# mrlooi/PoseCNN

Measured on AMD Instinct MI355X. Metric: frames/sec 640x480x21-class Hough-vote+RoI+ADD-loss, 1/2/4/8 MI355X, higher is better.
Workload: dtype f32 (FC GEMMs: exact 3-way split-bf16 x6 MFMA, products within 2^-24, fp32 accumulate: fp32-faithful)

## Files before the change

posecnn_amd/average_distance_loss/average_distance_loss_op.py:

```python
import warnings

import torch

from .. import _lib


def workspace_bytes(R, num_classes, num_points):
    return _lib.load().pcnn_add_loss_workspace_size(R, num_classes, num_points)


def search_stats(workspace, R, num_classes, num_points):
    off = _lib.load().pcnn_add_loss_stats_offset(R, num_classes, num_points)
    f, s, t = workspace[off:off + 12].cpu().view(torch.int32).tolist()
    return {"filter_items": f, "scan_items": s, "triples": t, "exact_evals": 16 * t}


def _workspace(what, ws, R, C, P):
    _lib.require(ws, torch.uint8, name=f"{what}: workspace")
    need = workspace_bytes(R, C, P)
    if ws.numel() < need:
        raise ValueError(f"{what}: workspace must hold {need} bytes, got {ws.numel()}")


def _models(what, points, symmetry, C, normalise):
    if normalise:
        points, symmetry = points.contiguous().float(), symmetry.contiguous().float()
    if points.dim() != 3 or points.shape[0] != C or points.shape[2] != 3:
        raise ValueError(f"{what}: points must be ({C}, P, 3), got {tuple(points.shape)}")
    _lib.require(points, torch.float32, name=f"{what}: points")
    _lib.require(symmetry, torch.float32, name=f"{what}: symmetry")
    if symmetry.numel() != C:
        raise ValueError(f"{what}: symmetry must have {C} elements, got {symmetry.numel()}")
    return points, symmetry


def average_distance_loss_prep(bottom_weight, bottom_symmetry, num_points, workspace, num_rois=None, points=None):
    if points is not None:
        warnings.warn("average_distance_loss_prep: `points` is ignored (the pruned ADD-S search is removed)",
                      DeprecationWarning, stacklevel=2)
    _lib.require_gpu(bottom_weight, bottom_symmetry, workspace)
    if bottom_weight.dim() != 2 or bottom_weight.shape[1] % 4:
        raise ValueError("average_distance_loss_prep: weight must be (R, 4C)")
    w = bottom_weight.contiguous().float()
    R, PC = w.shape
    sym = bottom_symmetry.contiguous().float()
    if sym.numel() != PC // 4:
        raise ValueError(f"average_distance_loss_prep: symmetry must have {PC // 4} elements, got {sym.numel()}")
    _workspace("average_distance_loss_prep", workspace, R, PC // 4, int(num_points))
    _lib.require_counter(num_rois, "average_distance_loss_prep: num_rois")
    rc = _lib.load().pcnn_add_loss_prep(_lib.ptr(w), _lib.ptr(sym), R,
                                        _lib.ptr(num_rois), PC // 4, int(num_points), _lib.ptr(workspace),
                                        workspace.numel(), _lib.stream_ptr())
    _lib.check(rc, "average_distance_loss_prep")


def average_distance_loss(bottom_prediction, bottom_target, bottom_weight, bottom_point, bottom_symmetry, margin,
                          name=None, num_rois=None, loss_norm_rows=0, loss_norm_rows_dev=None, out=None,
                          workspace=None, prepared=False):
    _lib.require_gpu(bottom_prediction, bottom_target, bottom_weight, bottom_point, bottom_symmetry)
    if margin < 0:
        raise ValueError(f"Need margin >= 0, got {margin}")
    what = "average_distance_loss"
    if bottom_prediction.dim() != 2 or bottom_prediction.shape[1] % 4:
        raise ValueError(f"{what}: prediction must be (R, 4C)")
    pred = bottom_prediction.contiguous().float()
    R, PC = pred.shape
    C = PC // 4
    for name, t in (("target", bottom_target), ("weight", bottom_weight)):
        if tuple(t.shape) != (R, PC):
            raise ValueError(f"{what}: {name} must be {(R, PC)} as the prediction, got {tuple(t.shape)}")
    points, symmetry = _models(what, bottom_point, bottom_symmetry, C, normalise=True)
    P = points.shape[1]
    _lib.require_counter(num_rois, f"{what}: num_rois")
    _lib.require_counter(loss_norm_rows_dev, f"{what}: loss_norm_rows_dev")
    if workspace is not None:
        _workspace(what, workspace, R, C, P)
    lib = _lib.load()
    if prepared and workspace is None:
        raise ValueError("prepared=True needs the workspace average_distance_loss_prep wrote")
    ws = workspace if workspace is not None else _lib.workspace(lib.pcnn_add_loss_workspace_size(R, C, P),
                                                                pred.device, "add_loss")
    if out is None:
        loss = torch.empty((1,), dtype=torch.float32, device=pred.device)
        diff = torch.empty((R, PC), dtype=torch.float32, device=pred.device)
    else:
        loss, diff = out
        _lib.require(loss, torch.float32, shape=(1,), name=f"{what}: out[0] (loss)")
        _lib.require(diff, torch.float32, shape=(R, PC), name=f"{what}: out[1] (bottom_diff)")
    fn = lib.pcnn_add_loss_fwd_prepared if prepared else lib.pcnn_add_loss_fwd
    rc = fn(_lib.ptr(pred), _lib.ptr(bottom_target.contiguous().float()), _lib.ptr(bottom_weight.contiguous().float()),
            _lib.ptr(points), _lib.ptr(symmetry), R,
            _lib.ptr(num_rois), C, P, float(margin), int(loss_norm_rows), _lib.ptr(loss_norm_rows_dev), _lib.ptr(loss),
            _lib.ptr(diff), _lib.ptr(ws), ws.numel(), _lib.stream_ptr())
    _lib.check(rc, "average_distance_loss")
    return loss, diff


def average_distance_loss_head_bwd(pred, target, weight, points, symmetry, margin, tanh_out, d_pred_scale, diff, dy8,
                                   workspace, num_rois=None, loss_norm_rows_dev=None, checked=True):
    _lib.require_gpu(pred, target, weight, points, symmetry, tanh_out, diff, dy8, workspace)
    what = "average_distance_loss_head_bwd"
    if margin < 0:
        raise ValueError(f"Need margin >= 0, got {margin}")
    if pred.dim() != 2 or pred.shape[1] % 4:
        raise ValueError(f"{what}: pred must be (R, 4C)")
    R, PC = pred.shape
    if PC > 256:
        raise ValueError(f"{what}: at most 256 columns (4C), got {PC}")
    _models(what, points, symmetry, PC // 4, normalise=False)
    if checked:
        for name, t in (("pred", pred), ("target", target), ("weight", weight), ("tanh_out", tanh_out),
                        ("diff", diff), ("dy8", dy8)):
            _lib.require(t, torch.float32, shape=(R, PC), name=f"{what}: {name}")
        if d_pred_scale is not None and _lib.require(d_pred_scale, torch.float32,
                                                     name=f"{what}: d_pred_scale").numel() < 1:
            raise ValueError(f"{what}: d_pred_scale needs one element")
        _workspace(what, workspace, R, PC // 4, points.shape[1])
        _lib.require_counter(num_rois, f"{what}: num_rois")
        _lib.require_counter(loss_norm_rows_dev, f"{what}: loss_norm_rows_dev")
    rc = _lib.load().pcnn_add_loss_fwd_head_bwd(
        _lib.ptr(pred), _lib.ptr(target), _lib.ptr(weight), _lib.ptr(points), _lib.ptr(symmetry), R,
        _lib.ptr(num_rois), PC // 4, points.shape[1], float(margin), 0, _lib.ptr(loss_norm_rows_dev), _lib.ptr(diff),
        _lib.ptr(workspace), workspace.numel(), _lib.ptr(tanh_out), _lib.ptr(d_pred_scale), _lib.ptr(dy8),
        _lib.stream_ptr())
    _lib.check(rc, "average_distance_loss_head_bwd")


def average_distance_loss_total(R, num_classes, num_points, workspace, loss, num_rois=None, checked=True):
    _lib.require_gpu(workspace, loss)
    if checked:
        _workspace("average_distance_loss_total", workspace, R, num_classes, num_points)
        _lib.require(loss, torch.float32, shape=(1,), name="average_distance_loss_total: loss")
        _lib.require_counter(num_rois, "average_distance_loss_total: num_rois")
    rc = _lib.load().pcnn_add_loss_total(R, _lib.ptr(num_rois), num_classes, num_points, _lib.ptr(workspace),
                                         workspace.numel(), _lib.ptr(loss), _lib.stream_ptr())
    _lib.check(rc, "average_distance_loss_total")


def average_distance_loss_grad(bottom_diff, grad, margin=0.01, name=None, num_rois=None, out=None):
    _lib.require_gpu(bottom_diff, grad)
    bd = bottom_diff.contiguous().float()
    g = grad.contiguous().float()
    if g.numel() < 1:
        raise ValueError("average_distance_loss_grad: grad needs one element")
    o = out if out is not None else torch.empty_like(bd)
    if out is not None:
        _lib.require(out, torch.float32, shape=tuple(bd.shape), name="average_distance_loss_grad: out")
    _lib.require_counter(num_rois, "average_distance_loss_grad: num_rois")
    rc = _lib.load().pcnn_add_loss_bwd(_lib.ptr(g), _lib.ptr(bd), bd.numel(),
                                       _lib.ptr(num_rois), bd.shape[-1], _lib.ptr(o), _lib.stream_ptr())
    _lib.check(rc, "average_distance_loss_grad")
    return o


class AverageDistanceFunction(torch.autograd.Function):

    @staticmethod
    def forward(ctx, pred, target, weight, points, symmetry, margin):
        loss, diff = average_distance_loss(pred, target, weight, points, symmetry, margin)
        ctx.save_for_backward(diff)
        ctx.margin = margin
        return loss

    @staticmethod
    def backward(ctx, grad):
        (diff,) = ctx.saved_tensors
        return average_distance_loss_grad(diff, grad.reshape(1), ctx.margin), None, None, None, None, None
```

posecnn_amd/csrc/average_distance.hip:

```cpp
#include "pcnn_common.h"
#include "head_common.h"
#include <atomic>
#include <cfloat>
#include <cstdlib>
#include <cstring>
#include <type_traits>

namespace {

#ifndef ADD_LANES
#define ADD_LANES 64
#endif
constexpr int kSymLanes = ADD_LANES;
#ifndef ADD_GRID
#define ADD_GRID 1024
#endif
#ifndef ADD_PPL
#define ADD_PPL 4
#endif
constexpr int kPPL = ADD_PPL;
constexpr int kPts = kSymLanes * kPPL;
constexpr int kMaxPointsLds = 8192;

__device__ __forceinline__ int rows_of(const int32_t* dev, int cap) {
  if (!dev) return cap;
  int r = *dev;
  return r < cap ? r : cap;
}

__device__ __forceinline__ void quat2rot(float s, float u, float v, float w, float* r) {
  r[0] = s * s + u * u - v * v - w * w;
  r[1] = 2 * (u * v - s * w);
  r[2] = 2 * (u * w + s * v);
  r[3] = 2 * (u * v + s * w);
  r[4] = s * s - u * u + v * v - w * w;
  r[5] = 2 * (v * w - s * u);
  r[6] = 2 * (u * w - s * v);
  r[7] = 2 * (v * w + s * u);
  r[8] = s * s - u * u - v * v + w * w;
}

__device__ __forceinline__ float div_rn(float x, float b, float r) {
  const float y0 = x * r;
  const float y1 = fmaf(fmaf(-y0, b, x), r, y0);
  return fmaf(fmaf(-y1, b, x), r, y1);
}
__device__ __forceinline__ double div_rn(double x, double b, double r) {
  const double y0 = x * r;
  const double y1 = fma(fma(-y0, b, x), r, y0);
  return fma(fma(-y1, b, x), r, y1);
}

__global__ void k_div_rn_check(const float* __restrict__ x, float b, int n, int dbl, float* __restrict__ out) {
  const int i = blockIdx.x * blockDim.x + threadIdx.x;
  if (i >= n) return;
  if (dbl) {
    const double bd = (double)b, rd = 1.0 / bd;
    out[i] = (float)div_rn((double)x[i], bd, rd);
  } else {
    out[i] = div_rn(x[i], b, 1.f / b);
  }
}

__device__ __forceinline__ int row_class(const float* __restrict__ weight, int n, int C) {
  const float* w = weight + (size_t)n * 4 * C;
  for (int i0 = 0; i0 < C; i0 += 8) {
    float v[8];
#pragma unroll
    for (int j = 0; j < 8; j++) v[j] = i0 + j < C ? w[4 * (i0 + j)] : 0.f;
#pragma unroll
    for (int j = 0; j < 8; j++)
      if (v[j] > 0) return i0 + j;
  }
  return -1;
}

__device__ __forceinline__ void add_point_terms(float X0, float X1, float X2, float x1, float y1, float z1, float x2,
                                                float y2, float z2, float s, float u, float v, float w, float margin,
                                                float bn, float rbn, double ln, double rln, float* acc) {
  const float dist = (x1 - x2) * (x1 - x2) + (y1 - y2) * (y1 - y2) + (z1 - z2) * (z1 - z2);
  if (dist < margin) return;
  acc[0] += (float)div_rn((double)(dist - margin), ln, rln);
  const float d0[9] = {2 * s, -2 * w, 2 * v, 2 * w, 2 * s, -2 * u, -2 * v, 2 * u, 2 * s};
  const float d1[9] = {2 * u, 2 * v, 2 * w, 2 * v, -2 * u, -2 * s, 2 * w, 2 * s, -2 * u};
  const float d2[9] = {-2 * v, 2 * u, 2 * s, 2 * u, 2 * v, 2 * w, -2 * s, 2 * w, -2 * v};
  const float d3[9] = {-2 * w, -2 * s, 2 * u, 2 * s, -2 * w, 2 * v, 2 * u, 2 * v, 2 * w};
  const float X[3] = {X0, X1, X2};
  const float df[3] = {x1 - x2, y1 - y2, z1 - z2};
  float e0 = 0.f, e1 = 0.f, e2 = 0.f, e3 = 0.f;
#pragma unroll
  for (int a = 0; a < 3; a++)
#pragma unroll
    for (int b = 0; b < 3; b++) {
      e0 += div_rn(df[a] * X[b] * d0[a * 3 + b], bn, rbn);
      e1 += div_rn(df[a] * X[b] * d1[a * 3 + b], bn, rbn);
      e2 += div_rn(df[a] * X[b] * d2[a * 3 + b], bn, rbn);
      e3 += div_rn(df[a] * X[b] * d3[a * 3 + b], bn, rbn);
    }
  acc[1] += e0; acc[2] += e1; acc[3] += e2; acc[4] += e3;
}

template <int kRows>
__device__ __forceinline__ void add_plain_rows(int n0, const float* __restrict__ pred,
                                               const float* __restrict__ target, const float* __restrict__ points,
                                               const float* __restrict__ symmetry, int R, int C, int P, float margin,
                                               int norm_rows, const int32_t* __restrict__ norm_rows_dev, int nchunk,
                                               const int32_t* __restrict__ rcls, float* __restrict__ partial,
                                               float (*red)[5]) {
  const int half = kRows == 2 ? (int)(threadIdx.x / kPts) : 0, tid = (int)(threadIdx.x % kPts);
  const int n = n0 + half;
  const bool live = n < R;
  const int cls = live ? rcls[n] : -1;
  const bool sym = cls >= 0 && symmetry[cls] > 0;
  float* out = partial + (size_t)(live ? n : 0) * nchunk * 5;
  if (live && !sym)
    for (int i = tid; i < nchunk * 5; i += kPts) out[i] = 0.f;
  const bool work = live && !sym && cls >= 0;
  float acc[5] = {0.f, 0.f, 0.f, 0.f, 0.f};
  if (work) {
    const int PC = 4 * C;
    const float* tq = target + (size_t)n * PC + 4 * cls;
    const float* pq = pred + (size_t)n * PC + 4 * cls;
    float Rg[9], Rp[9];
    quat2rot(tq[0], tq[1], tq[2], tq[3], Rg);
    const float s = pq[0], u = pq[1], v = pq[2], w = pq[3];
    quat2rot(s, u, v, w, Rp);
    const int Rn = norm_rows_dev ? *norm_rows_dev : (norm_rows > 0 ? norm_rows : R);
    const float bn = (float)(Rn * P), rbn = 1.f / bn;
    const double ln = 2.0 * (double)Rn * (double)P, rln = 1.0 / ln;
    const float* pts = points + (size_t)cls * P * 3;
    for (int p = tid; p < P; p += kPts) {
      const float X0 = pts[p * 3 + 0], X1 = pts[p * 3 + 1], X2 = pts[p * 3 + 2];
      const float x1 = Rp[0] * X0 + Rp[1] * X1 + Rp[2] * X2;
      const float y1 = Rp[3] * X0 + Rp[4] * X1 + Rp[5] * X2;
      const float z1 = Rp[6] * X0 + Rp[7] * X1 + Rp[8] * X2;
      const float x2 = Rg[0] * X0 + Rg[1] * X1 + Rg[2] * X2;
      const float y2 = Rg[3] * X0 + Rg[4] * X1 + Rg[5] * X2;
      const float z2 = Rg[6] * X0 + Rg[7] * X1 + Rg[8] * X2;
      add_point_terms(X0, X1, X2, x1, y1, z1, x2, y2, z2, s, u, v, w, margin, bn, rbn, ln, rln, acc);
    }
  }
#pragma unroll
  for (int q = 0; q < 5; q++) acc[q] = pcnn::wave_sum(acc[q]);
  if (pcnn::lane_id() == 0)
    for (int q = 0; q < 5; q++) red[threadIdx.x >> 6][q] = acc[q];
  __syncthreads();
  if (work && tid < 5) {
    float t = 0.f;
    for (int i = 0; i < kPts / 64; i++) t += red[half * (kPts / 64) + i][tid];
    out[tid] = t;
  }
}

#ifndef ADD_GROUPS
#define ADD_GROUPS 4
#endif
constexpr int kSymGroups = ADD_GROUPS;
constexpr int kSymThreads = kSymLanes * kSymGroups;
#ifndef ADD_BLK
#define ADD_BLK 8
#endif
constexpr int kBlk = ADD_BLK;

typedef unsigned u32x4 __attribute__((ext_vector_type(4)));
typedef float f32x16 __attribute__((ext_vector_type(16)));
typedef __bf16 bf16x8 __attribute__((ext_vector_type(8)));

constexpr int kFiltWaves = 8;
constexpr int kFiltThreads = 64 * kFiltWaves;
constexpr int kFiltMaxPoints = 2816;
constexpr int kFiltList = 1024;
constexpr int kFiltBlk = ((kFiltMaxPoints + 31) / 32 + kFiltWaves - 1) / kFiltWaves;
constexpr float kFiltWin = 2.8e-4f;
constexpr float kFiltM2Min = 0x1p-40f, kFiltM2Max = 0x1p40f;
constexpr unsigned kFiltPadNorm = 0x7180u;

template <bool F>
struct FiltLds {};
template <>
struct FiltLds<true> {
  float4 sq[kPts];
  float smin[kFiltWaves][kPts];
  unsigned long long skey[kPts];
  unsigned list[kFiltList];
  int cnt, m2;
};

__device__ __forceinline__ unsigned bf16_rn(float x) {
  const unsigned b = __float_as_uint(x);
  return (b + 0x7fffu + ((b >> 16) & 1u)) >> 16;
}
__device__ __forceinline__ float bf16_val(unsigned h) { return __uint_as_float(h << 16); }
__device__ __forceinline__ void bf16_split2(float x, unsigned& h, unsigned& m) {
  h = bf16_rn(x);
  m = bf16_rn(x - bf16_val(h));
}

__device__ __forceinline__ void filt_candidate(const float4& c, float n, u32x4& k0, u32x4& k8) {
  unsigned xh, xm, yh, ym, zh, zm;
  bf16_split2(c.x, xh, xm);
  bf16_split2(c.y, yh, ym);
  bf16_split2(c.z, zh, zm);
  const unsigned nh = bf16_rn(n);
  const float r1 = n - bf16_val(nh);
  const unsigned nm = bf16_rn(r1);
  const unsigned nl = bf16_rn(r1 - bf16_val(nm));
  k0 = (u32x4){xh | xh << 16, xm | xm << 16, yh | yh << 16, ym | ym << 16};
  k8 = (u32x4){zh | zh << 16, zm | zm << 16, nh | nm << 16, nl};
}

__device__ __forceinline__ float filt_min17(float m, const f32x16& v) {
  float a = fminf(fminf(v[0], v[1]), v[2]);
  float b = fminf(fminf(v[3], v[4]), v[5]);
  a = fminf(fminf(a, v[6]), v[7]);
  b = fminf(fminf(b, v[8]), v[9]);
  a = fminf(fminf(a, v[10]), v[11]);
  b = fminf(fminf(b, v[12]), v[13]);
  a = fminf(fminf(a, v[14]), v[15]);
  return fminf(fminf(m, a), b);
}

template <int NF>
__device__ __forceinline__ int filter_search(FiltLds<true>& fl, const float4* gpts, const char* cimg, int P, int nq,
                                             float win, int* s_imin) {
  const int lane = pcnn::lane_id(), r = lane & 31, h = lane >> 5;
  const int wave = __builtin_amdgcn_readfirstlane((int)(threadIdx.x >> 6));
  const int nblk = (P + 31) >> 5, bq = nblk / kFiltWaves, brem = nblk % kFiltWaves;
  const int b0 = wave * bq + min(wave, brem), b1 = b0 + bq + (wave < brem ? 1 : 0);
  bf16x8 qb[NF];
#pragma unroll
  for (int f = 0; f < NF; f++) {
    const float4 q = fl.sq[f * 32 + r];
    unsigned xh, xm, yh, ym, zh, zm;
    bf16_split2(-2.f * q.x, xh, xm);
    bf16_split2(-2.f * q.y, yh, ym);
    bf16_split2(-2.f * q.z, zh, zm);
    const u32x4 w = h == 0 ? (u32x4){xh | xm << 16, xh | xm << 16, yh | ym << 16, yh | ym << 16}
                           : (u32x4){zh | zm << 16, zh | zm << 16, 0x3f803f80u, 0x00003f80u};
    qb[f] = __builtin_bit_cast(bf16x8, w);
  }
  const f32x16 zero = {0.f, 0.f, 0.f, 0.f, 0.f, 0.f, 0.f, 0.f, 0.f, 0.f, 0.f, 0.f, 0.f, 0.f, 0.f, 0.f};
  const char* ap = cimg + r * 32 + h * 16;
  float bmin[kFiltBlk][NF];
  bf16x8 a = *(const bf16x8*)(ap + min(b0, nblk - 1) * 1024);
#pragma unroll
  for (int k = 0; k < kFiltBlk; k++) {
    if (b0 + k < b1) {
      const bf16x8 an = *(const bf16x8*)(ap + min(b0 + k + 1, nblk - 1) * 1024);
      f32x16 v = __builtin_amdgcn_mfma_f32_32x32x16_bf16(a, qb[0], zero, 0, 0, 0);
#pragma unroll
      for (int f = 0; f < NF; f++) {
        f32x16 vn = v;
        if (f + 1 < NF) vn = __builtin_amdgcn_mfma_f32_32x32x16_bf16(a, qb[f + 1], zero, 0, 0, 0);
        __builtin_amdgcn_sched_barrier(0);
        bmin[k][f] = filt_min17(FLT_MAX, v);
        __builtin_amdgcn_sched_barrier(0);
        v = vn;
      }
      a = an;
    } else {
#pragma unroll
      for (int f = 0; f < NF; f++) bmin[k][f] = FLT_MAX;
    }
  }
#pragma unroll
  for (int f = 0; f < NF; f++) {
    float m = bmin[0][f];
#pragma unroll
    for (int k = 1; k < kFiltBlk; k++) m = fminf(m, bmin[k][f]);
    m = fminf(m, __shfl_xor(m, 32, 64));
    if (h == 0) fl.smin[wave][f * 32 + r] = m;
  }
  __syncthreads();
  unsigned mask[NF];
#pragma unroll
  for (int f = 0; f < NF; f++) {
    float t = fl.smin[0][f * 32 + r];
#pragma unroll
    for (int g = 1; g < kFiltWaves; g++) t = fminf(t, fl.smin[g][f * 32 + r]);
    const float thr = t + win;
    unsigned mk = 0u;
#pragma unroll
    for (int k = 0; k < kFiltBlk; k++) mk |= bmin[k][f] <= thr ? 1u << k : 0u;
    mask[f] = mk;
  }
#pragma unroll
  for (int f = 0; f < NF; f++)
    if (f * 32 + r >= nq) mask[f] = 0u;
  int nrec = 0;
  for (;;) {
    int mine = 0;
#pragma unroll
    for (int f = 0; f < NF; f++) mine += __popc(mask[f]);
    int incl = mine;
#pragma unroll
    for (int o = 1; o < 64; o <<= 1) {
      const int t = __shfl_up(incl, o, 64);
      if (lane >= o) incl += t;
    }
    const int total = __shfl(incl, 63, 64);
    int base = 0;
    if (lane == 0 && total > 0) base = atomicAdd(&fl.cnt, total);
    int pos = __shfl(base, 0, 64) + incl - mine;
    int pending = 0;
#pragma unroll
    for (int f = 0; f < NF; f++) {
      unsigned mk = mask[f];
      while (mk && pos < kFiltList) {
        const int bit = __ffs(mk) - 1;
        mk &= mk - 1;
        fl.list[pos++] = (unsigned)(f * 32 + r) << 16 | (unsigned)(b0 + bit) << 1 | (unsigned)h;
      }
      mask[f] = mk;
      pending |= mk != 0u;
    }
    __syncthreads();
    const int n = min(fl.cnt, kFiltList);
    for (int w = threadIdx.x; w < n; w += blockDim.x) {
      const unsigned rec = fl.list[w];
      const int qi = rec >> 16;
      const int i0 = (int)((rec >> 1) & 0x7fffu) * 32 + 4 * (int)(rec & 1u);
      const float4 q = fl.sq[qi];
      unsigned long long best = ~0ull;
#pragma unroll
      for (int reg = 0; reg < 16; reg++) {
        const int idx = i0 + (reg & 3) + 8 * (reg >> 2);
        const float4 c = gpts[min(idx, P - 1)];
        const float d = (q.x - c.x) * (q.x - c.x) + (q.y - c.y) * (q.y - c.y) + (q.z - c.z) * (q.z - c.z);
        const unsigned long long key = (unsigned long long)__float_as_uint(d) << 32 | (unsigned long long)(unsigned)idx;
        if (idx < P && d < FLT_MAX && key < best) best = key;
      }
      if (best != ~0ull) atomicMin(&fl.skey[qi], best);
    }
    nrec += n;
    pending = __syncthreads_or(pending);
    if (!pending) break;
    if (threadIdx.x == 0) fl.cnt = 0;
    __syncthreads();
  }
  if (threadIdx.x < kPts) {
    const unsigned long long key = fl.skey[threadIdx.x];
    s_imin[threadIdx.x] = key == ~0ull ? -1 : (int)(unsigned)(key & 0xffffffffull);
  }
  return nrec;
}

template <bool kFilt>
__global__ void __launch_bounds__(kFilt ? kFiltThreads : kSymThreads) k_add_rows(const float* __restrict__ pred,
                                                           const float* __restrict__ target,
                                                           const float* __restrict__ weight,
                                                           const float* __restrict__ points,
                                                           const float* __restrict__ symmetry, int R_cap,
                                                           const int32_t* __restrict__ num_rois_dev, int C, int P,
                                                           float margin, int norm_rows,
                                                           const int32_t* __restrict__ norm_rows_dev, int nchunk,
                                                           const int32_t* __restrict__ rcls,
                                                           const int32_t* __restrict__ sym_rows,
                                                           const int32_t* __restrict__ nsym,
                                                           int32_t* __restrict__ queue,
                                                           int32_t* __restrict__ stats,
                                                           float* __restrict__ partial) {
  extern __shared__ __attribute__((aligned(16))) float4 gpts[];
  __shared__ FiltLds<kFilt> fl;
  __shared__ float mdist[kSymGroups - 1][kPts];
  __shared__ int midx[kSymGroups - 1][kPts];
  __shared__ float red[(kFilt ? kFiltThreads : kSymThreads) / 64][5];
  __shared__ int s_imin[kPts];
  const int R = rows_of(num_rois_dev, R_cap);
  const int sym_items = *nsym * nchunk;
  constexpr int kPlain = kFilt ? kFiltThreads / kPts : 1;
  const int items = sym_items + (R + kPlain - 1) / kPlain;
  const int grp = threadIdx.x / kSymLanes, lt = threadIdx.x % kSymLanes;
  const int quarter = ((P + kSymGroups - 1) / kSymGroups + kBlk - 1) / kBlk * kBlk;
  const int c0 = grp * quarter, c1 = min(P, c0 + quarter);
  __shared__ int s_item;
  int st_filter = 0, st_scan = 0, st_triples = 0;
  for (;;) {
  __syncthreads();
  if (threadIdx.x == 0) {
    s_item = atomicAdd(queue, 1);
    if constexpr (kFilt) { fl.cnt = 0; fl.m2 = 0; }
  }
  __syncthreads();
  const int item = s_item;
  if (item >= items) break;
  if (item >= sym_items) {
    add_plain_rows<kPlain>((item - sym_items) * kPlain, pred, target, points, symmetry, R, C, P, margin, norm_rows,
                           norm_rows_dev, nchunk, rcls, partial, red);
    continue;
  }
  const int nfull = P / kPts, nsym_rows = *nsym;
  int n, chunk, slot;
  if (item < nsym_rows * nfull) {
    slot = item / nfull;
    chunk = item % nfull;
  } else {
    slot = item - nsym_rows * nfull;
    chunk = nfull;
  }
  n = sym_rows[slot];
  const int PC = 4 * C;
  const int cls = rcls[n];
  float* out = partial + ((size_t)n * nchunk + chunk) * 5;
  const float* tq = target + (size_t)n * PC + 4 * cls;
  const float* pq = pred + (size_t)n * PC + 4 * cls;
  float Rg[9], Rp[9];
  quat2rot(tq[0], tq[1], tq[2], tq[3], Rg);
  const float s = pq[0], u = pq[1], v = pq[2], w = pq[3];
  quat2rot(s, u, v, w, Rp);
  const float* pts = points + (size_t)cls * P * 3;
  const int nq = min(kPts, P - chunk * kPts);
  bool searched = false;
  int nrec = 0;
  float Xt0 = 0.f, Xt1 = 0.f, Xt2 = 0.f;
  if constexpr (kFilt) {
    char* cimg = (char*)gpts + (((size_t)P * sizeof(float4) + 31) & ~(size_t)31);
    const int Ppad = (P + 31) & ~31;
    float mx = 0.f;
    int bad = 0;
    constexpr int kStage = (kFiltMaxPoints + kFiltThreads - 1) / kFiltThreads;
    float Xs[kStage][3];
#pragma unroll
    for (int k = 0; k < kStage; k++) {
      const int i = (int)threadIdx.x + k * kFiltThreads;
      const int ii = i < P ? i : 0;
      Xs[k][0] = pts[ii * 3 + 0]; Xs[k][1] = pts[ii * 3 + 1]; Xs[k][2] = pts[ii * 3 + 2];
    }
#pragma unroll
    for (int k = 0; k < kStage; k++) {
      const int i = (int)threadIdx.x + k * kFiltThreads;
      if (i >= Ppad) continue;
      u32x4 k0 = {0u, 0u, 0u, 0u}, k8 = {0u, 0u, kFiltPadNorm, 0u};
      if (i < P) {
        const float X0 = Xs[k][0], X1 = Xs[k][1], X2 = Xs[k][2];
        const float4 c = make_float4(Rg[0] * X0 + Rg[1] * X1 + Rg[2] * X2, Rg[3] * X0 + Rg[4] * X1 + Rg[5] * X2,
                                     Rg[6] * X0 + Rg[7] * X1 + Rg[8] * X2, 0.f);
        gpts[i] = c;
        const float nn = c.x * c.x + c.y * c.y + c.z * c.z;
        bad |= !(nn <= kFiltM2Max);
        mx = fmaxf(mx, nn);
        filt_candidate(c, nn, k0, k8);
      }
      *(u32x4*)(cimg + (size_t)i * 32) = k0;
      *(u32x4*)(cimg + (size_t)i * 32 + 16) = k8;
    }
    if (threadIdx.x < kPts) {
      const int p = chunk * kPts + (int)threadIdx.x;
      const int pp = p < P ? p : 0;
      const float X0 = pts[pp * 3 + 0], X1 = pts[pp * 3 + 1], X2 = pts[pp * 3 + 2];
      Xt0 = X0; Xt1 = X1; Xt2 = X2;
      const float4 q = make_float4(Rp[0] * X0 + Rp[1] * X1 + Rp[2] * X2, Rp[3] * X0 + Rp[4] * X1 + Rp[5] * X2,
                                   Rp[6] * X0 + Rp[7] * X1 + Rp[8] * X2, 0.f);
      fl.sq[threadIdx.x] = q;
      const float nn = q.x * q.x + q.y * q.y + q.z * q.z;
      bad |= !(nn <= kFiltM2Max);
      mx = fmaxf(mx, nn);
      fl.skey[threadIdx.x] = ~0ull;
    }
    mx = pcnn::wave_max(mx);
    if (pcnn::lane_id() == 0) atomicMax(&fl.m2, __float_as_int(mx));
    bad = __syncthreads_or(bad);
    const float m2 = __int_as_float(fl.m2);
    if (!bad && m2 >= kFiltM2Min) {
      nrec = nq > 64 ? filter_search<8>(fl, gpts, cimg, P, nq, kFiltWin * m2, s_imin)
                     : filter_search<2>(fl, gpts, cimg, P, nq, kFiltWin * m2, s_imin);
      searched = true;
    }
  } else {
  for (int i = threadIdx.x; i < P; i += blockDim.x) {
    const float X0 = pts[i * 3 + 0], X1 = pts[i * 3 + 1], X2 = pts[i * 3 + 2];
    gpts[i] = make_float4(Rg[0] * X0 + Rg[1] * X1 + Rg[2] * X2, Rg[3] * X0 + Rg[4] * X1 + Rg[5] * X2,
                          Rg[6] * X0 + Rg[7] * X1 + Rg[8] * X2, 0.f);
  }
  __syncthreads();
  }
  if (!searched) {
  float qx[kPPL], qy[kPPL], qz[kPPL], Xq[kPPL][3];
  int pq_[kPPL];
#pragma unroll
  for (int k = 0; k < kPPL; k++) {
    const int p = chunk * kPts + k * kSymLanes + lt;
    pq_[k] = p;
    const int pp = p < P ? p : 0;
    Xq[k][0] = pts[pp * 3 + 0]; Xq[k][1] = pts[pp * 3 + 1]; Xq[k][2] = pts[pp * 3 + 2];
    qx[k] = Rp[0] * Xq[k][0] + Rp[1] * Xq[k][1] + Rp[2] * Xq[k][2];
    qy[k] = Rp[3] * Xq[k][0] + Rp[4] * Xq[k][1] + Rp[5] * Xq[k][2];
    qz[k] = Rp[6] * Xq[k][0] + Rp[7] * Xq[k][1] + Rp[8] * Xq[k][2];
  }
  auto dist_to = [&](int k, const float4& c) {
    return (qx[k] - c.x) * (qx[k] - c.x) + (qy[k] - c.y) * (qy[k] - c.y) + (qz[k] - c.z) * (qz[k] - c.z);
  };
  float dmin[kPPL];
  int iblk[kPPL];
#pragma unroll
  for (int k = 0; k < kPPL; k++) { dmin[k] = FLT_MAX; iblk[k] = -1; }
  typedef float f2 __attribute__((ext_vector_type(2)));
  f2 px[kPPL / 2], py[kPPL / 2], pz[kPPL / 2];
#pragma unroll
  for (int h = 0; h < kPPL / 2; h++) {
    px[h] = (f2){qx[2 * h], qx[2 * h + 1]};
    py[h] = (f2){qy[2 * h], qy[2 * h + 1]};
    pz[h] = (f2){qz[2 * h], qz[2 * h + 1]};
  }
  auto scan = [&](auto np_c) {
    constexpr int NP = decltype(np_c)::value;
    int i = c0;
    for (; i + kBlk <= c1; i += kBlk) {
      float4 c[kBlk];
#pragma unroll
      for (int j = 0; j < kBlk; j++) c[j] = gpts[i + j];
#pragma unroll
      for (int h = 0; h < NP; h++) {
        f2 d[kBlk];
#pragma unroll
        for (int j = 0; j < kBlk; j++) {
          const f2 ex = px[h] - c[j].x, ey = py[h] - c[j].y, ez = pz[h] - c[j].z;
          d[j] = ex * ex + ey * ey + ez * ez;
        }
#pragma unroll
        for (int e = 0; e < 2; e++) {
          const int k = 2 * h + e;
          float bm = fminf(d[0][e], d[1][e]);
#pragma unroll
          for (int j = 2; j < kBlk; j += 2) bm = fminf(bm, fminf(d[j][e], d[j + 1][e]));
          if (bm < dmin[k]) { dmin[k] = bm; iblk[k] = i; }
        }
      }
    }
    for (; i < c1; i++) {
      const float4 c = gpts[i];
#pragma unroll
      for (int k = 0; k < 2 * NP; k++) {
        const float d = dist_to(k, c);
        if (d < dmin[k]) { dmin[k] = d; iblk[k] = i; }
      }
    }
  };
  if (nq > 2 * kSymLanes) scan(std::integral_constant<int, kPPL / 2>{});
  else scan(std::integral_constant<int, 1>{});
  if (grp > 0 && grp < kSymGroups) {
#pragma unroll
    for (int k = 0; k < kPPL; k++) {
      mdist[grp - 1][k * kSymLanes + lt] = dmin[k];
      midx[grp - 1][k * kSymLanes + lt] = iblk[k];
    }
  }
  __syncthreads();
  if (grp == 0) {
#pragma unroll
    for (int k = 0; k < kPPL; k++) {
#pragma unroll
      for (int g = 0; g < kSymGroups - 1; g++) {
        const float d = mdist[g][k * kSymLanes + lt];
        if (d < dmin[k]) { dmin[k] = d; iblk[k] = midx[g][k * kSymLanes + lt]; }
      }
      int im = -1;
      if (iblk[k] >= 0) {
        const int e = min(iblk[k] + kBlk, P);
        for (int j = iblk[k]; j < e; j++)
          if (dist_to(k, gpts[j]) == dmin[k]) { im = j; break; }
      }
      s_imin[k * kSymLanes + lt] = im;
    }
  }
  }
  __syncthreads();
  float acc[5] = {0.f, 0.f, 0.f, 0.f, 0.f};
  for (int jj = threadIdx.x; jj < kPts; jj += blockDim.x) {
    const int p = chunk * kPts + jj;
    if (p >= P) continue;
    const int im = s_imin[jj] < 0 ? p : s_imin[jj];
    static_assert(kPts == kSymThreads, "one tail point per thread: jj == threadIdx.x");
    const float X0 = kFilt ? Xt0 : pts[p * 3 + 0], X1 = kFilt ? Xt1 : pts[p * 3 + 1], X2 = kFilt ? Xt2 : pts[p * 3 + 2];
    const float x1 = Rp[0] * X0 + Rp[1] * X1 + Rp[2] * X2;
    const float y1 = Rp[3] * X0 + Rp[4] * X1 + Rp[5] * X2;
    const float z1 = Rp[6] * X0 + Rp[7] * X1 + Rp[8] * X2;
    const float4 cm = gpts[im];
    const int Rn = norm_rows_dev ? *norm_rows_dev : (norm_rows > 0 ? norm_rows : R);
    const float bn = (float)(Rn * P), rbn = 1.f / bn;
    const double ln = 2.0 * (double)Rn * (double)P, rln = 1.0 / ln;
    add_point_terms(X0, X1, X2, x1, y1, z1, cm.x, cm.y, cm.z, s, u, v, w, margin, bn, rbn, ln, rln, acc);
  }
#pragma unroll
  for (int q = 0; q < 5; q++) acc[q] = pcnn::wave_sum(acc[q]);
  if (pcnn::lane_id() == 0 && threadIdx.x < kSymThreads)
    for (int q = 0; q < 5; q++) red[threadIdx.x >> 6][q] = acc[q];
  __syncthreads();
  if (threadIdx.x < 5) {
    float t = 0.f;
    for (int i = 0; i < kSymThreads / 64; i++) t += red[i][threadIdx.x];
    out[threadIdx.x] = t;
  }
  if (searched) {
    st_filter++;
    st_triples += nrec;
  } else {
    st_scan++;
  }
  __syncthreads();
  }
  if (threadIdx.x == 0) {
    if (st_filter) atomicAdd(stats + 0, st_filter);
    if (st_scan) atomicAdd(stats + 1, st_scan);
    if (st_triples) atomicAdd(stats + 2, st_triples);
  }
}

__global__ void __launch_bounds__(1024) k_add_prep(const float* __restrict__ weight, const float* __restrict__ symmetry,
                                                    int R_cap, const int32_t* __restrict__ num_rois_dev, int C,
                                                    int32_t* __restrict__ rcls, int32_t* __restrict__ sym_rows,
                                                    int32_t* __restrict__ nsym, int32_t* __restrict__ queue,
                                                    int32_t* __restrict__ stats) {
  __shared__ int wcount[16];
  __shared__ int base;
  const int R = rows_of(num_rois_dev, R_cap);
  const int lane = pcnn::lane_id(), wave = threadIdx.x >> 6;
  if (threadIdx.x == 0) base = 0;
  __syncthreads();
  for (int n0 = 0; n0 < R; n0 += blockDim.x) {
    const int n = n0 + threadIdx.x;
    int cls = -1;
    if (n < R) {
      cls = row_class(weight, n, C);
      rcls[n] = cls;
    }
    const bool sym = n < R && cls >= 0 && symmetry[cls] > 0;
    const uint64_t m = __ballot(sym);
    if (lane == 0) wcount[wave] = __popcll(m);
    __syncthreads();
    int off = base;
    for (int w = 0; w < wave; w++) off += wcount[w];
    if (sym) sym_rows[off + __popcll(m & pcnn::lanemask_lt())] = n;
    __syncthreads();
    if (threadIdx.x == 0) {
      int t = 0;
      for (int w = 0; w < (int)(blockDim.x >> 6); w++) t += wcount[w];
      base += t;
    }
    __syncthreads();
  }
  if (threadIdx.x == 0) {
    *nsym = base;
    *queue = 0;
    stats[0] = stats[1] = stats[2] = 0;
  }
}

__device__ __forceinline__ void fold_row(int n, int nchunk, const float* __restrict__ partial, int lane, float* s) {
#pragma unroll
  for (int q = 0; q < 5; q++) s[q] = 0.f;
  for (int k = lane; k < nchunk; k += 64)
    for (int q = 0; q < 5; q++) s[q] += partial[((size_t)n * nchunk + k) * 5 + q];
#pragma unroll
  for (int q = 0; q < 5; q++) s[q] = pcnn::wave_sum(s[q]);
}

__device__ __forceinline__ void finish_row(int n, int R, int C, int nchunk, const int32_t* __restrict__ rcls,
                                           const float* __restrict__ partial, float* __restrict__ row_loss,
                                           float* __restrict__ bottom_diff, int lane) {
  if (n >= R) return;
  const int cls = rcls[n];
  float s[5];
  fold_row(n, nchunk, partial, lane, s);
  const int PC = 4 * C;
  for (int col = lane; col < PC; col += 64) {
    float vv = 0.f;
    if (cls >= 0 && col >= 4 * cls && col < 4 * cls + 4) vv = s[1 + col - 4 * cls];
    bottom_diff[(size_t)n * PC + col] = vv;
  }
  if (lane == 0) row_loss[n] = cls >= 0 ? s[0] : 0.f;
}

__global__ void __launch_bounds__(256) k_add_finish_rows(int R_cap, const int32_t* __restrict__ num_rois_dev, int C,
                                                          int nchunk, const int32_t* __restrict__ rcls,
                                                          const float* __restrict__ partial,
                                                          float* __restrict__ row_loss,
                                                          float* __restrict__ bottom_diff) {
  const int R = rows_of(num_rois_dev, R_cap);
  const int n = (blockIdx.x * blockDim.x + threadIdx.x) >> 6;
  finish_row(n, R, C, nchunk, rcls, partial, row_loss, bottom_diff, pcnn::lane_id());
}

__global__ void __launch_bounds__(256) k_add_finish_head(int R_cap, const int32_t* __restrict__ num_rois_dev, int C,
                                                          int nchunk, const int32_t* __restrict__ rcls,
                                                          const float* __restrict__ partial,
                                                          float* __restrict__ row_loss,
                                                          float* __restrict__ bottom_diff,
                                                          const float* __restrict__ t_in,
                                                          const float* __restrict__ pw,
                                                          const float* __restrict__ pred,
                                                          const float* __restrict__ dscale, float* __restrict__ dy8) {
  const int R = rows_of(num_rois_dev, R_cap);
  const int n = (blockIdx.x * blockDim.x + threadIdx.x) >> 6;
  const int lane = pcnn::lane_id();
  if (n >= R) return;
  const int cls = rcls[n];
  float s[5];
  fold_row(n, nchunk, partial, lane, s);
  const int PC = 4 * C;
  const float g = dscale ? dscale[0] : 1.f;
  float dp[4];
#pragma unroll
  for (int k = 0; k < 4; k++) {
    const int col = lane + 64 * k;
    float vv = 0.f;
    if (cls >= 0 && col >= 4 * cls && col < 4 * cls + 4) vv = s[1 + col - 4 * cls];
    if (col < PC) bottom_diff[(size_t)n * PC + col] = vv;
    dp[k] = col < PC ? g * vv : 0.f;
  }
  if (lane == 0) row_loss[n] = cls >= 0 ? s[0] : 0.f;
  pcnn_head::head_bwd_row(dp, t_in, pw, pred, n, PC, lane, dy8);
}

__global__ void __launch_bounds__(1024) k_add_total(int R_cap, const int32_t* __restrict__ num_rois_dev,
                                                     const float* __restrict__ row_loss, float* __restrict__ loss) {
  __shared__ float red[16];
  const int R = rows_of(num_rois_dev, R_cap);
  float my = 0.f;
  for (int n = threadIdx.x; n < R; n += blockDim.x) my += row_loss[n];
  my = pcnn::wave_sum(my);
  if (pcnn::lane_id() == 0) red[threadIdx.x >> 6] = my;
  __syncthreads();
  if (threadIdx.x == 0) {
    float t = 0.f;
    for (int i = 0; i < (int)(blockDim.x >> 6); i++) t += red[i];
    loss[0] = t;
  }
}

__global__ void k_add_bwd(const float* __restrict__ top_diff, const float* __restrict__ bottom_diff, int n,
                          float* __restrict__ out) {
  const float g = top_diff[0];
  for (int i = blockIdx.x * blockDim.x + threadIdx.x; i < n; i += gridDim.x * blockDim.x) out[i] = g * bottom_diff[i];
}

__global__ void k_add_bwd_rows(const float* __restrict__ top_diff, const float* __restrict__ bottom_diff,
                               const int32_t* __restrict__ num_rois_dev, int R_cap, int row_len,
                               float* __restrict__ out) {
  const float g = top_diff[0];
  const int n = rows_of(num_rois_dev, R_cap) * row_len;
  for (int i = blockIdx.x * blockDim.x + threadIdx.x; i < n; i += gridDim.x * blockDim.x) out[i] = g * bottom_diff[i];
}

}

extern "C" int pcnn_div_rn_check(const float* x, float b, int n, int dbl, float* out, void* stream) {
  PCNN_REQUIRE(x && out && n >= 0 && b != 0.f);
  if (n == 0) return PCNN_OK;
  hipLaunchKernelGGL(k_div_rn_check, dim3((n + 255) / 256), dim3(256), 0, (hipStream_t)stream, x, b, n, dbl, out);
  PCNN_CHECK_LAUNCH();
  return PCNN_OK;
}

struct AddWs {
  float* partial;
  int32_t *rcls, *sym_rows, *nsym, *queue;
  float* row_loss;
  int32_t* stats;
  size_t stats_off;
};
static AddWs add_carve(void* workspace, int R_cap, int P, size_t* bytes) {
  const int nchunk = (P + kPts - 1) / kPts;
  const size_t R = (size_t)(R_cap > 0 ? R_cap : 1);
  pcnn::Carve cv(workspace);
  AddWs w;
  w.partial = cv.take<float>(R * nchunk * 5);
  w.rcls = cv.take<int32_t>(R);
  w.sym_rows = cv.take<int32_t>(R);
  w.nsym = cv.take<int32_t>(1);
  w.queue = cv.take<int32_t>(1);
  w.row_loss = cv.take<float>(R);
  w.stats = cv.take<int32_t>(4);
  w.stats_off = cv.off - 4 * sizeof(int32_t);
  if (bytes) *bytes = cv.off + 256;
  return w;
}

extern "C" size_t pcnn_add_loss_workspace_size(int R_cap, int C, int P) {
  (void)C;
  size_t b = 0;
  (void)add_carve(nullptr, R_cap, P, &b);
  return b;
}

static void add_launch_prep(const AddWs& w, const float* weight, const float* symmetry, int R_cap,
                            const int32_t* num_rois_dev, int C, hipStream_t st) {
  hipLaunchKernelGGL(k_add_prep, dim3(1), dim3(1024), 0, st, weight, symmetry, R_cap, num_rois_dev, C, w.rcls,
                     w.sym_rows, w.nsym, w.queue, w.stats);
}

static size_t add_filter_lds(int P) {
  return (((size_t)P * sizeof(float4) + 31) & ~(size_t)31) + (size_t)((P + 31) & ~31) * 32;
}

static bool add_use_filter(int P) {
  const char* mode = getenv("PCNN_ADD_SEARCH");
  if (mode && strcmp(mode, "scan") == 0) return false;
  if (P > kFiltMaxPoints) return false;
  static std::atomic<int> room[pcnn::kMaxDevices];
  int dev = 0;
  if (hipGetDevice(&dev) != hipSuccess || dev < 0 || dev >= pcnn::kMaxDevices) return false;
  int have = room[dev].load(std::memory_order_acquire);
  if (have == 0) {
    hipFuncAttributes fa;
    int lds = 0;
    have = -1;
    if (hipFuncGetAttributes(&fa, (const void*)k_add_rows<true>) == hipSuccess &&
        hipDeviceGetAttribute(&lds, hipDeviceAttributeMaxSharedMemoryPerBlock, dev) == hipSuccess &&
        lds > (int)fa.sharedSizeBytes) {
      const int dyn = lds - (int)fa.sharedSizeBytes;
      if (hipFuncSetAttribute((const void*)k_add_rows<true>, hipFuncAttributeMaxDynamicSharedMemorySize, dyn) ==
          hipSuccess)
        have = dyn;
    }
    if (have < 0) (void)hipGetLastError();
    room[dev].store(have, std::memory_order_release);
  }
  return have > 0 && add_filter_lds(P) <= (size_t)have;
}

static void add_launch_rows(const AddWs& w, const float* pred, const float* target, const float* weight,
                            const float* points, const float* symmetry, int R_cap, const int32_t* num_rois_dev,
                            int C, int P, float margin, int loss_norm_rows, const int32_t* loss_norm_rows_dev,
                            hipStream_t st) {
  const int nchunk = (P + kPts - 1) / kPts;
  const long items = (long)R_cap * nchunk + R_cap;
  const int grid = (int)(items < ADD_GRID ? items : ADD_GRID);
  if (add_use_filter(P))
    hipLaunchKernelGGL(k_add_rows<true>, dim3(grid), dim3(kFiltThreads), add_filter_lds(P), st, pred, target, weight,
                       points, symmetry, R_cap, num_rois_dev, C, P, margin, loss_norm_rows, loss_norm_rows_dev,
                       nchunk, w.rcls, w.sym_rows, w.nsym, w.queue, w.stats, w.partial);
  else
    hipLaunchKernelGGL(k_add_rows<false>, dim3(grid), dim3(kSymThreads), (size_t)P * sizeof(float4), st, pred,
                       target, weight, points, symmetry, R_cap, num_rois_dev, C, P, margin, loss_norm_rows,
                       loss_norm_rows_dev, nchunk, w.rcls, w.sym_rows, w.nsym, w.queue, w.stats, w.partial);
}

static int add_loss_fwd(const float* pred, const float* target, const float* weight, const float* points,
                        const float* symmetry, int R_cap, const int32_t* num_rois_dev, int C, int P, float margin,
                        int loss_norm_rows, const int32_t* loss_norm_rows_dev, float* loss, float* bottom_diff,
                        void* workspace, size_t workspace_bytes, bool prepared, void* stream) {
  PCNN_REQUIRE(pred && target && weight && points && symmetry && loss && bottom_diff && workspace);
  PCNN_REQUIRE(R_cap > 0 && C > 0 && P > 0 && P <= kMaxPointsLds);
  if (workspace_bytes < pcnn_add_loss_workspace_size(R_cap, C, P)) return PCNN_ECAPACITY;
  hipStream_t st = (hipStream_t)stream;
  const int nchunk = (P + kPts - 1) / kPts;
  const AddWs w = add_carve(workspace, R_cap, P, nullptr);
  if (!prepared) add_launch_prep(w, weight, symmetry, R_cap, num_rois_dev, C, st);
  add_launch_rows(w, pred, target, weight, points, symmetry, R_cap, num_rois_dev, C, P, margin, loss_norm_rows,
                  loss_norm_rows_dev, st);
  hipLaunchKernelGGL(k_add_finish_rows, dim3((R_cap + 3) / 4), dim3(256), 0, st, R_cap, num_rois_dev, C, nchunk,
                     w.rcls, w.partial, w.row_loss, bottom_diff);
  hipLaunchKernelGGL(k_add_total, dim3(1), dim3(1024), 0, st, R_cap, num_rois_dev, w.row_loss, loss);
  PCNN_CHECK_LAUNCH();
  return PCNN_OK;
}

extern "C" size_t pcnn_add_loss_stats_offset(int R_cap, int C, int P) {
  (void)C;
  return add_carve(nullptr, R_cap, P, nullptr).stats_off;
}

extern "C" int pcnn_add_loss_fwd(const float* pred, const float* target, const float* weight, const float* points,
                                 const float* symmetry, int R_cap, const int32_t* num_rois_dev, int C, int P,
                                 float margin, int loss_norm_rows, const int32_t* loss_norm_rows_dev, float* loss,
                                 float* bottom_diff, void* workspace, size_t workspace_bytes, void* stream) {
  return add_loss_fwd(pred, target, weight, points, symmetry, R_cap, num_rois_dev, C, P, margin, loss_norm_rows,
                      loss_norm_rows_dev, loss, bottom_diff, workspace, workspace_bytes, false, stream);
}

extern "C" int pcnn_add_loss_prep(const float* weight, const float* symmetry, int R_cap, const int32_t* num_rois_dev,
                                  int C, int P, void* workspace, size_t workspace_bytes, void* stream) {
  PCNN_REQUIRE(weight && symmetry && workspace && R_cap > 0 && C > 0 && P > 0 && P <= kMaxPointsLds);
  if (workspace_bytes < pcnn_add_loss_workspace_size(R_cap, C, P)) return PCNN_ECAPACITY;
  const AddWs w = add_carve(workspace, R_cap, P, nullptr);
  add_launch_prep(w, weight, symmetry, R_cap, num_rois_dev, C, (hipStream_t)stream);
  PCNN_CHECK_LAUNCH();
  return PCNN_OK;
}

extern "C" int pcnn_add_loss_fwd_prepared(const float* pred, const float* target, const float* weight,
                                          const float* points, const float* symmetry, int R_cap,
                                          const int32_t* num_rois_dev, int C, int P, float margin,
                                          int loss_norm_rows, const int32_t* loss_norm_rows_dev, float* loss,
                                          float* bottom_diff, void* workspace, size_t workspace_bytes,
                                          void* stream) {
  return add_loss_fwd(pred, target, weight, points, symmetry, R_cap, num_rois_dev, C, P, margin, loss_norm_rows,
                      loss_norm_rows_dev, loss, bottom_diff, workspace, workspace_bytes, true, stream);
}

extern "C" int pcnn_add_loss_fwd_head_bwd(const float* pred, const float* target, const float* weight,
                                          const float* points, const float* symmetry, int R_cap,
                                          const int32_t* num_rois_dev, int C, int P, float margin,
                                          int loss_norm_rows, const int32_t* loss_norm_rows_dev, float* bottom_diff,
                                          void* workspace, size_t workspace_bytes, const float* tanh_out,
                                          const float* d_pred_scale, float* d_y8, void* stream) {
  PCNN_REQUIRE(pred && target && weight && points && symmetry && bottom_diff && workspace && tanh_out && d_y8);
  PCNN_REQUIRE(R_cap > 0 && C > 0 && 4 * C <= 256 && P > 0 && P <= kMaxPointsLds);
  if (workspace_bytes < pcnn_add_loss_workspace_size(R_cap, C, P)) return PCNN_ECAPACITY;
  hipStream_t st = (hipStream_t)stream;
  const int nchunk = (P + kPts - 1) / kPts;
  const AddWs w = add_carve(workspace, R_cap, P, nullptr);
  add_launch_rows(w, pred, target, weight, points, symmetry, R_cap, num_rois_dev, C, P, margin, loss_norm_rows,
                  loss_norm_rows_dev, st);
  pcnn::launch_last(k_add_finish_head, dim3((R_cap + 3) / 4), dim3(256), 0, st, R_cap, num_rois_dev, C, nchunk,
                     w.rcls, w.partial, w.row_loss, bottom_diff, tanh_out, weight, pred, d_pred_scale, d_y8);
  PCNN_CHECK_LAUNCH();
  return PCNN_OK;
}

extern "C" int pcnn_add_loss_total(int R_cap, const int32_t* num_rois_dev, int C, int P, const void* workspace,
                                   size_t workspace_bytes, float* loss, void* stream) {
  PCNN_REQUIRE(workspace && loss && R_cap > 0 && C > 0 && P > 0);
  if (workspace_bytes < pcnn_add_loss_workspace_size(R_cap, C, P)) return PCNN_ECAPACITY;
  const AddWs w = add_carve(const_cast<void*>(workspace), R_cap, P, nullptr);
  hipLaunchKernelGGL(k_add_total, dim3(1), dim3(1024), 0, (hipStream_t)stream, R_cap, num_rois_dev, w.row_loss,
                     loss);
  PCNN_CHECK_LAUNCH();
  return PCNN_OK;
}

extern "C" int pcnn_add_loss_bwd(const float* top_diff, const float* bottom_diff, int n,
                                 const int32_t* num_rois_dev, int row_len, float* out, void* stream) {
  PCNN_REQUIRE(top_diff && bottom_diff && out && n >= 0);
  hipStream_t st = (hipStream_t)stream;
  if (n == 0) return PCNN_OK;
  const int blocks = (n + 255) / 256 < 1024 ? (n + 255) / 256 : 1024;
  if (num_rois_dev) {
    PCNN_REQUIRE(row_len > 0);
    hipLaunchKernelGGL(k_add_bwd_rows, dim3(blocks), dim3(256), 0, st, top_diff, bottom_diff, num_rois_dev,
                       n / row_len, row_len, out);
  } else {
    hipLaunchKernelGGL(k_add_bwd, dim3(blocks), dim3(256), 0, st, top_diff, bottom_diff, n, out);
  }
  PCNN_CHECK_LAUNCH();
  return PCNN_OK;
}
```

Measured before the change: 4563.

## Assign contiguous symmetric-row chunk ranges per block and reuse staged candidate image

In the filtered ADD-S kernel, each block now takes a static, cost-weighted contiguous range of (row, chunk) items instead of pulling every item from the atomic queue, with the queue kept for leftover plain rows. Because consecutive chunks of the same row stay on one block, the staged candidate point image, and its max-norm and bad flags, is rebuilt only when the class or target quaternion changes. The filter grid is sized to the CU count, with an environment cap. This removes repeated staging and per-item atomics, but static partitioning can unbalance load, and the per-item LDS flag resets and stats bookkeeping are now more intricate.

```diff
diff --git a/posecnn_amd/average_distance_loss/average_distance_loss_op.py b/posecnn_amd/average_distance_loss/average_distance_loss_op.py
--- a/posecnn_amd/average_distance_loss/average_distance_loss_op.py
+++ b/posecnn_amd/average_distance_loss/average_distance_loss_op.py
@@ -11,8 +11,8 @@
 
 def search_stats(workspace, R, num_classes, num_points):
     off = _lib.load().pcnn_add_loss_stats_offset(R, num_classes, num_points)
-    f, s, t = workspace[off:off + 12].cpu().view(torch.int32).tolist()
-    return {"filter_items": f, "scan_items": s, "triples": t, "exact_evals": 16 * t}
+    f, s, t, g = workspace[off:off + 16].cpu().view(torch.int32).tolist()
+    return {"filter_items": f, "scan_items": s, "triples": t, "exact_evals": 16 * t, "image_stagings": g}
 
 
 def _workspace(what, ws, R, C, P):
diff --git a/posecnn_amd/csrc/average_distance.hip b/posecnn_amd/csrc/average_distance.hip
--- a/posecnn_amd/csrc/average_distance.hip
+++ b/posecnn_amd/csrc/average_distance.hip
@@ -183,8 +183,27 @@
   float smin[kFiltWaves][kPts];
   unsigned long long skey[kPts];
   unsigned list[kFiltList];
-  int cnt, m2;
+  int cnt;
+  int m2, qbad;
+  int cm2, cbad;
 };
+
+#ifndef ADD_COST_FULL
+#define ADD_COST_FULL 8
+#endif
+#ifndef ADD_COST_SHORT
+#define ADD_COST_SHORT 4
+#endif
+constexpr int kCostFull = ADD_COST_FULL, kCostShort = ADD_COST_SHORT;
+
+__device__ __forceinline__ int range_start(int b, int W, int nsym, int P, int nchunk) {
+  const int nfull = P / kPts;
+  const long long row = (long long)nfull * kCostFull + (P % kPts ? kCostShort : 0);
+  const long long t = ((long long)b * row * nsym + W - 1) / W;
+  const int slot = (int)(t / row);
+  const int chunk = (int)((t % row + kCostFull - 1) / kCostFull);
+  return slot * nchunk + min(chunk, nchunk);
+}
 
 __device__ __forceinline__ unsigned bf16_rn(float x) {
   const unsigned b = __float_as_uint(x);
@@ -374,23 +393,62 @@
   const int quarter = ((P + kSymGroups - 1) / kSymGroups + kBlk - 1) / kBlk * kBlk;
   const int c0 = grp * quarter, c1 = min(P, c0 + quarter);
   __shared__ int s_item;
-  int st_filter = 0, st_scan = 0, st_triples = 0;
+  int st_filter = 0, st_scan = 0, st_triples = 0, st_stage = 0;
+  int n = 0, cls = 0, chunk = 0;
+  float Rg[9], Rp[9], s = 0.f, u = 0.f, v = 0.f, w = 0.f;
+  const float* pts = points;
+  int pair = 0, pair_end = 0, cur_slot = -1, img_cls = -1, cand_m2 = 0, cand_bad = 0;
+  unsigned img_q[4] = {0u, 0u, 0u, 0u};
+  if constexpr (kFilt) {
+    const int nsym_rows = *nsym;
+    pair = range_start((int)blockIdx.x, (int)gridDim.x, nsym_rows, P, nchunk);
+    pair_end = range_start((int)blockIdx.x + 1, (int)gridDim.x, nsym_rows, P, nchunk);
+    if (threadIdx.x == 0) { fl.cnt = 0; fl.m2 = 0; fl.qbad = 0; fl.cm2 = 0; fl.cbad = 0; }
+    __syncthreads();
+  }
   for (;;) {
-  __syncthreads();
-  if (threadIdx.x == 0) {
-    s_item = atomicAdd(queue, 1);
-    if constexpr (kFilt) { fl.cnt = 0; fl.m2 = 0; }
-  }
-  __syncthreads();
-  const int item = s_item;
-  if (item >= items) break;
+  int item;
+  if (kFilt && pair < pair_end) {
+    item = pair++;
+  } else {
+    __syncthreads();
+    if (threadIdx.x == 0) s_item = (kFilt ? sym_items : 0) + atomicAdd(queue, 1);
+    __syncthreads();
+    item = s_item;
+    if (item >= items) break;
+  }
   if (item >= sym_items) {
     add_plain_rows<kPlain>((item - sym_items) * kPlain, pred, target, points, symmetry, R, C, P, margin, norm_rows,
                            norm_rows_dev, nchunk, rcls, partial, red);
     continue;
   }
+  const int PC = 4 * C;
+  bool stage = false;
+  if constexpr (kFilt) {
+    const int slot = item / nchunk;
+    chunk = item - slot * nchunk;
+    if (slot != cur_slot) {
+      cur_slot = slot;
+      n = sym_rows[slot];
+      cls = rcls[n];
+      const float* tq = target + (size_t)n * PC + 4 * cls;
+      const float* pq = pred + (size_t)n * PC + 4 * cls;
+      const float t0 = tq[0], t1 = tq[1], t2 = tq[2], t3 = tq[3];
+      s = pq[0]; u = pq[1]; v = pq[2]; w = pq[3];
+      quat2rot(s, u, v, w, Rp);
+      pts = points + (size_t)cls * P * 3;
+      const unsigned q0 = __float_as_uint(t0), q1 = __float_as_uint(t1), q2 = __float_as_uint(t2),
+                     q3 = __float_as_uint(t3);
+      stage = cls != img_cls || q0 != img_q[0] || q1 != img_q[1] || q2 != img_q[2] || q3 != img_q[3];
+      if (stage) {
+        img_cls = cls;
+        img_q[0] = q0; img_q[1] = q1; img_q[2] = q2; img_q[3] = q3;
+        quat2rot(t0, t1, t2, t3, Rg);
+      }
+    }
+  } else {
   const int nfull = P / kPts, nsym_rows = *nsym;
-  int n, chunk, slot;
+  int slot;
   if (item < nsym_rows * nfull) {
     slot = item / nfull;
     chunk = item % nfull;
@@ -399,16 +457,15 @@
     chunk = nfull;
   }
   n = sym_rows[slot];
-  const int PC = 4 * C;
-  const int cls = rcls[n];
-  float* out = partial + ((size_t)n * nchunk + chunk) * 5;
+  cls = rcls[n];
   const float* tq = target + (size_t)n * PC + 4 * cls;
   const float* pq = pred + (size_t)n * PC + 4 * cls;
-  float Rg[9], Rp[9];
   quat2rot(tq[0], tq[1], tq[2], tq[3], Rg);
-  const float s = pq[0], u = pq[1], v = pq[2], w = pq[3];
+  s = pq[0]; u = pq[1]; v = pq[2]; w = pq[3];
   quat2rot(s, u, v, w, Rp);
-  const float* pts = points + (size_t)cls * P * 3;
+  pts = points + (size_t)cls * P * 3;
+  }
+  float* out = partial + ((size_t)n * nchunk + chunk) * 5;
   const int nq = min(kPts, P - chunk * kPts);
   bool searched = false;
   int nrec = 0;
@@ -418,6 +475,7 @@
     const int Ppad = (P + 31) & ~31;
     float mx = 0.f;
     int bad = 0;
+    if (stage) {
     constexpr int kStage = (kFiltMaxPoints + kFiltThreads - 1) / kFiltThreads;
     float Xs[kStage][3];
 #pragma unroll
@@ -444,6 +502,13 @@
       *(u32x4*)(cimg + (size_t)i * 32) = k0;
       *(u32x4*)(cimg + (size_t)i * 32 + 16) = k8;
     }
+    mx = pcnn::wave_max(mx);
+    if (pcnn::lane_id() == 0) atomicMax(&fl.cm2, __float_as_int(mx));
+    if (bad) fl.cbad = 1;
+    mx = 0.f;
+    bad = 0;
+    st_stage++;
+    }
     if (threadIdx.x < kPts) {
       const int p = chunk * kPts + (int)threadIdx.x;
       const int pp = p < P ? p : 0;
@@ -459,8 +524,11 @@
     }
     mx = pcnn::wave_max(mx);
     if (pcnn::lane_id() == 0) atomicMax(&fl.m2, __float_as_int(mx));
-    bad = __syncthreads_or(bad);
-    const float m2 = __int_as_float(fl.m2);
+    if (bad) fl.qbad = 1;
+    __syncthreads();
+    if (stage) { cand_m2 = fl.cm2; cand_bad = fl.cbad; }
+    bad = cand_bad | fl.qbad;
+    const float m2 = __int_as_float(max(cand_m2, fl.m2));
     if (!bad && m2 >= kFiltM2Min) {
       nrec = nq > 64 ? filter_search<8>(fl, gpts, cimg, P, nq, kFiltWin * m2, s_imin)
                      : filter_search<2>(fl, gpts, cimg, P, nq, kFiltWin * m2, s_imin);
@@ -591,6 +659,9 @@
     for (int i = 0; i < kSymThreads / 64; i++) t += red[i][threadIdx.x];
     out[threadIdx.x] = t;
   }
+  if constexpr (kFilt) {
+    if (threadIdx.x == 0) { fl.cnt = 0; fl.m2 = 0; fl.qbad = 0; fl.cm2 = 0; fl.cbad = 0; }
+  }
   if (searched) {
     st_filter++;
     st_triples += nrec;
@@ -603,6 +674,7 @@
     if (st_filter) atomicAdd(stats + 0, st_filter);
     if (st_scan) atomicAdd(stats + 1, st_scan);
     if (st_triples) atomicAdd(stats + 2, st_triples);
+    if (st_stage) atomicAdd(stats + 3, st_stage);
   }
 }
 
@@ -642,7 +714,7 @@
   if (threadIdx.x == 0) {
     *nsym = base;
     *queue = 0;
-    stats[0] = stats[1] = stats[2] = 0;
+    stats[0] = stats[1] = stats[2] = stats[3] = 0;
   }
 }
 
@@ -819,6 +891,27 @@
   return have > 0 && add_filter_lds(P) <= (size_t)have;
 }
 
+static int add_filter_grid(long items) {
+  static std::atomic<int> cus[pcnn::kMaxDevices];
+  int dev = 0, n = ADD_GRID;
+  if (hipGetDevice(&dev) == hipSuccess && dev >= 0 && dev < pcnn::kMaxDevices) {
+    int have = cus[dev].load(std::memory_order_acquire);
+    if (have == 0) {
+      have = -1;
+      int c = 0;
+      if (hipDeviceGetAttribute(&c, hipDeviceAttributeMultiprocessorCount, dev) == hipSuccess && c > 0) have = c;
+      else (void)hipGetLastError();
+      cus[dev].store(have, std::memory_order_release);
+    }
+    if (have > 0) n = have;
+  }
+  if (const char* cap = getenv("PCNN_ADD_GRID")) {
+    const long c = strtol(cap, nullptr, 10);
+    if (c >= 1 && c < n) n = (int)c;
+  }
+  return (int)(items < n ? items : n);
+}
+
 static void add_launch_rows(const AddWs& w, const float* pred, const float* target, const float* weight,
                             const float* points, const float* symmetry, int R_cap, const int32_t* num_rois_dev,
                             int C, int P, float margin, int loss_norm_rows, const int32_t* loss_norm_rows_dev,
@@ -827,8 +920,8 @@
   const long items = (long)R_cap * nchunk + R_cap;
   const int grid = (int)(items < ADD_GRID ? items : ADD_GRID);
   if (add_use_filter(P))
-    hipLaunchKernelGGL(k_add_rows<true>, dim3(grid), dim3(kFiltThreads), add_filter_lds(P), st, pred, target, weight,
-                       points, symmetry, R_cap, num_rois_dev, C, P, margin, loss_norm_rows, loss_norm_rows_dev,
+    hipLaunchKernelGGL(k_add_rows<true>, dim3(add_filter_grid(items)), dim3(kFiltThreads), add_filter_lds(P), st, pred,
+                       target, weight, points, symmetry, R_cap, num_rois_dev, C, P, margin, loss_norm_rows, loss_norm_rows_dev,
                        nchunk, w.rcls, w.sym_rows, w.nsym, w.queue, w.stats, w.partial);
   else
     hipLaunchKernelGGL(k_add_rows<false>, dim3(grid), dim3(kSymThreads), (size_t)P * sizeof(float4), st, pred,
```

New measurement: 4610 (median of 6 runs). 1.0% higher.
